# jy0205/Pyramid-Flow

Hardware: NVIDIA H100
Metric: dit_step_latent_tokens_per_sec (higher is better)
Workload: dtype bf16

## Files before the change

pyramid_flow_b200/csrc/pf_attn.cu:

```cuda
#include <algorithm>
#include <vector>

#include "../../include/pf_b200.h"
#include "pf_common.cuh"

namespace pf {

constexpr int ATT_BM = 128;
constexpr int ATT_BN = 128;
constexpr int ATT_HD = 64;
constexpr int ATT_STAGES = 2;
constexpr int ATT_THREADS = 384;
constexpr int ATT_TILE_BYTES = ATT_BN * ATT_HD * 2;
constexpr int ATT_SMEM_BYTES = (1 + 2 * ATT_STAGES) * ATT_TILE_BYTES + 1024;

struct AttnArgs {
  __nv_bfloat16* out;
  long long ldo;
  int batch, heads, seq, q_tiles;
  float scale_log2;
  const int* seg;
  const int* time;
  const int* sched;
  int sched_stride;
  __nv_bfloat16* peer_out[PF_MAX_PEERS];
  int peer_count, peer_chunk_rows, peer_col_begin;
};

__global__ void __launch_bounds__(ATT_THREADS, 1)
attn_fwd_kernel(const __grid_constant__ CUtensorMap tm_q, const __grid_constant__ CUtensorMap tm_k,
                const __grid_constant__ CUtensorMap tm_v, const AttnArgs a) {
  extern __shared__ uint8_t smem_raw[];
  uint8_t* smem = reinterpret_cast<uint8_t*>((reinterpret_cast<uintptr_t>(smem_raw) + 1023) & ~uintptr_t(1023));
  uint8_t* smem_q = smem;
  uint8_t* smem_k = smem + ATT_TILE_BYTES;
  uint8_t* smem_v = smem_k + ATT_STAGES * ATT_TILE_BYTES;

  __shared__ __align__(8) uint64_t bar_q;
  __shared__ __align__(8) uint64_t k_full[ATT_STAGES], k_empty[ATT_STAGES], v_full[ATT_STAGES], v_empty[ATT_STAGES];

  const int warp = threadIdx.x >> 5;
  const int lane = threadIdx.x & 31;
  const int wgroup = warp >> 2;
  const int qt = a.q_tiles - 1 - static_cast<int>(blockIdx.x);
  const int h = blockIdx.y;
  const int b = blockIdx.z;
  const int bh = b * a.heads + h;
  const int* sched = a.sched + (static_cast<size_t>(b) * a.q_tiles + qt) * a.sched_stride;
  const int n_kv = sched[0];

  if (threadIdx.x == 0) {
    tma_prefetch_desc(&tm_q);
    tma_prefetch_desc(&tm_k);
    tma_prefetch_desc(&tm_v);
    mbar_init(&bar_q, 1);
    for (int i = 0; i < ATT_STAGES; ++i) {
      mbar_init(&k_full[i], 1);
      mbar_init(&k_empty[i], 8);
      mbar_init(&v_full[i], 1);
      mbar_init(&v_empty[i], 8);
    }
    fence_barrier_init();
  }
  __syncthreads();

  if (wgroup == 0) {
    setmaxnreg_dec<40>();
    if (warp == 0 && elect_one()) {
      mbar_arrive_expect_tx(&bar_q, ATT_TILE_BYTES);
      tma_load_3d(smem_q, &tm_q, &bar_q, 0, qt * ATT_BM, bh);
      int st = 0;
      uint32_t ph = 0;
      for (int j = 0; j < n_kv; ++j) {
        const int kt = sched[1 + j] >> 1;
        mbar_wait(&k_empty[st], ph ^ 1);
        mbar_arrive_expect_tx(&k_full[st], ATT_TILE_BYTES);
        tma_load_3d(smem_k + st * ATT_TILE_BYTES, &tm_k, &k_full[st], 0, kt * ATT_BN, bh);
        mbar_wait(&v_empty[st], ph ^ 1);
        mbar_arrive_expect_tx(&v_full[st], ATT_TILE_BYTES);
        tma_load_3d(smem_v + st * ATT_TILE_BYTES, &tm_v, &v_full[st], 0, kt * ATT_BN, bh);
        if (++st == ATT_STAGES) {
          st = 0;
          ph ^= 1;
        }
      }
    }
    return;
  }

  setmaxnreg_inc<232>();
  const int wg = wgroup - 1;
  const int g4 = lane >> 2, t4 = lane & 3;
  const int row0 = wg * 64 + (warp & 3) * 16 + g4;
  const float c = a.scale_log2;
  const int* sg = a.seg + static_cast<size_t>(b) * a.seq;
  const int* tm = a.time + static_cast<size_t>(b) * a.seq;
  int seg_q[2], time_q[2];
#pragma unroll
  for (int r = 0; r < 2; ++r) {
    const int qpos = qt * ATT_BM + row0 + 8 * r;
    const bool q_valid = qpos < a.seq;
    seg_q[r] = q_valid ? sg[qpos] : -0x7fffffff;
    time_q[r] = q_valid ? tm[qpos] : -0x7fffffff;
  }
  float m_run[2] = {-INFINITY, -INFINITY};
  float l_run[2] = {0.f, 0.f};
  float o[32];
#pragma unroll
  for (int i = 0; i < 32; ++i) o[i] = 0.f;

  mbar_wait(&bar_q, 0);
  const uint64_t dq = make_smem_desc_kmajor_sw128(smem_u32(smem_q) + wg * (64 * 128));
  int st = 0;
  uint32_t ph = 0;
  for (int j = 0; j < n_kv; ++j) {
    const int entry = sched[1 + j];
    const int kt = entry >> 1;
    const bool masked = (entry & 1) != 0;

    float s[64];
    mbar_wait(&k_full[st], ph);
    {
      const uint64_t dk = make_smem_desc_kmajor_sw128(smem_u32(smem_k + st * ATT_TILE_BYTES));
      wgmma_fence();
#pragma unroll
      for (int kk = 0; kk < ATT_HD / 16; ++kk) wgmma_ss_n128(s, dq + 2 * kk, dk + 2 * kk, kk != 0 ? 1u : 0u);
      wgmma_commit();
      wgmma_wait<0>();
      wgmma_reg_fence(s);
    }
    if (lane == 0) mbar_arrive(&k_empty[st]);

    if (masked) {
#pragma unroll
      for (int i = 0; i < 16; ++i) {
#pragma unroll
        for (int e = 0; e < 2; ++e) {
          const int kv = kt * ATT_BN + 8 * i + 2 * t4 + e;
          int sk = 0x7fffffff, tk = 0x7fffffff;
          if (kv < a.seq) {
            sk = __ldg(sg + kv);
            tk = __ldg(tm + kv);
          }
          if (!(sk == seg_q[0] && tk <= time_q[0])) s[4 * i + e] = -INFINITY;
          if (!(sk == seg_q[1] && tk <= time_q[1])) s[4 * i + 2 + e] = -INFINITY;
        }
      }
    }

    float alpha[2];
#pragma unroll
    for (int r = 0; r < 2; ++r) {
      float mx = -INFINITY;
#pragma unroll
      for (int i = 0; i < 16; ++i) mx = fmaxf(mx, fmaxf(s[4 * i + 2 * r], s[4 * i + 2 * r + 1]));
      mx = fmaxf(mx, __shfl_xor_sync(0xffffffffu, mx, 1));
      mx = fmaxf(mx, __shfl_xor_sync(0xffffffffu, mx, 2));
      const float m_new = fmaxf(m_run[r], mx);
      alpha[r] = (m_new == -INFINITY) ? 1.f : ex2_approx_f((m_run[r] - m_new) * c);
      m_run[r] = m_new;
      const float m_ref = (m_new == -INFINITY) ? 0.f : m_new * c;
      float sum = 0.f;
#pragma unroll
      for (int i = 0; i < 16; ++i) {
        const float p0 = ex2_approx_f(fmaf(s[4 * i + 2 * r], c, -m_ref));
        const float p1 = ex2_approx_f(fmaf(s[4 * i + 2 * r + 1], c, -m_ref));
        s[4 * i + 2 * r] = p0;
        s[4 * i + 2 * r + 1] = p1;
        sum += p0 + p1;
      }
      l_run[r] = l_run[r] * alpha[r] + sum;
    }
#pragma unroll
    for (int i = 0; i < 8; ++i) {
      o[4 * i + 0] *= alpha[0];
      o[4 * i + 1] *= alpha[0];
      o[4 * i + 2] *= alpha[1];
      o[4 * i + 3] *= alpha[1];
    }

    mbar_wait(&v_full[st], ph);
    {
      const uint32_t sv = smem_u32(smem_v + st * ATT_TILE_BYTES);
      uint32_t pa[ATT_BN / 16][4];
#pragma unroll
      for (int kk = 0; kk < ATT_BN / 16; ++kk) {
        pa[kk][0] = pack_bf16x2(s[8 * kk + 0], s[8 * kk + 1]);
        pa[kk][1] = pack_bf16x2(s[8 * kk + 2], s[8 * kk + 3]);
        pa[kk][2] = pack_bf16x2(s[8 * kk + 4], s[8 * kk + 5]);
        pa[kk][3] = pack_bf16x2(s[8 * kk + 6], s[8 * kk + 7]);
      }
      wgmma_reg_fence(o);
      wgmma_fence();
#pragma unroll
      for (int kk = 0; kk < ATT_BN / 16; ++kk) {
        const uint64_t dv = make_smem_desc(sv + kk * 2048, ATT_BN * 128, 1024);
        wgmma_rs_n64_tb(o, pa[kk], dv);
      }
      wgmma_commit();
      wgmma_wait<0>();
      wgmma_reg_fence(o);
    }
    if (lane == 0) mbar_arrive(&v_empty[st]);
    if (++st == ATT_STAGES) {
      st = 0;
      ph ^= 1;
    }
  }

#pragma unroll
  for (int r = 0; r < 2; ++r) {
    float l = l_run[r];
    l += __shfl_xor_sync(0xffffffffu, l, 1);
    l += __shfl_xor_sync(0xffffffffu, l, 2);
    const float inv = (l > 0.f) ? 1.f / l : 0.f;
    const int qpos = qt * ATT_BM + row0 + 8 * r;
    if (qpos >= a.seq) continue;
    __nv_bfloat16* dst;
    if (a.peer_count > 1) {
      const int pr = qpos / a.peer_chunk_rows;
      dst = a.peer_out[pr] + static_cast<size_t>(qpos - pr * a.peer_chunk_rows) * a.ldo + a.peer_col_begin + h * ATT_HD;
    } else {
      dst = a.out + (static_cast<size_t>(b) * a.seq + qpos) * a.ldo + h * ATT_HD;
    }
#pragma unroll
    for (int i = 0; i < 8; ++i)
      *reinterpret_cast<uint32_t*>(dst + 8 * i + 2 * t4) = pack_bf16x2(o[4 * i + 2 * r] * inv, o[4 * i + 2 * r + 1] * inv);
  }
}

int warmup_attn() {
  return ensure_dyn_smem(reinterpret_cast<const void*>(attn_fwd_kernel), ATT_SMEM_BYTES, "attn_fwd_kernel");
}

}

extern "C" int pf_attn_build_schedule(const int32_t* seg, const int32_t* time, int32_t batch, int32_t seq,
                                      int32_t* out, int64_t* allowed_pairs) {
  using namespace pf;
  PF_REQUIRE(batch > 0 && seq > 0, "pf_attn_build_schedule: bad shape");
  const int tiles = (seq + 127) / 128;
  const int stride = 1 + tiles;
  if (out == nullptr) return stride;
  PF_REQUIRE(seg && time, "pf_attn_build_schedule: null ids");
  for (int b = 0; b < batch; ++b) {
    const int32_t* sg = seg + static_cast<size_t>(b) * seq;
    const int32_t* tm = time + static_cast<size_t>(b) * seq;
    std::vector<int32_t> tmin(tiles), tmax(tiles), smin(tiles), smax(tiles);
    for (int t = 0; t < tiles; ++t) {
      const int lo = t * 128, hi = std::min(seq, lo + 128);
      int32_t a = tm[lo], bq = tm[lo], c = sg[lo], d = sg[lo];
      for (int i = lo; i < hi; ++i) {
        a = std::min(a, tm[i]);
        bq = std::max(bq, tm[i]);
        c = std::min(c, sg[i]);
        d = std::max(d, sg[i]);
      }
      tmin[t] = a; tmax[t] = bq; smin[t] = c; smax[t] = d;
    }
    int64_t pairs = 0;
    for (int qt = 0; qt < tiles; ++qt) {
      int32_t* row = out + (static_cast<size_t>(b) * tiles + qt) * stride;
      int cnt = 0;
      const int qlo = qt * 128, qhi = std::min(seq, qlo + 128);
      for (int kt = 0; kt < tiles; ++kt) {
        const int klo = kt * 128, khi = std::min(seq, klo + 128);
        if (tmax[qt] < tmin[kt]) continue;
        if (smax[qt] < smin[kt] || smax[kt] < smin[qt]) continue;
        const bool uniform = (smin[qt] == smax[qt]) && (smin[kt] == smax[kt]) && (smin[qt] == smin[kt]);
        const bool full = uniform && (tmin[qt] >= tmax[kt]) && (khi - klo == 128);
        int64_t n_allowed = 0;
        if (full) {
          n_allowed = static_cast<int64_t>(qhi - qlo) * (khi - klo);
        } else {
          for (int i = qlo; i < qhi; ++i)
            for (int j = klo; j < khi; ++j) n_allowed += (sg[i] == sg[j] && tm[i] >= tm[j]) ? 1 : 0;
          if (n_allowed == 0) continue;
        }
        pairs += n_allowed;
        row[1 + cnt] = (kt << 1) | (full ? 0 : 1);
        ++cnt;
      }
      row[0] = cnt;
      for (int i = 1 + cnt; i < stride; ++i) row[i] = 0;
    }
    if (allowed_pairs) allowed_pairs[b] = pairs;
  }
  return stride;
}

extern "C" int pf_attn_fwd_masked(const pf_attn_desc* d, void* stream_) {
  using namespace pf;
  cudaStream_t stream = static_cast<cudaStream_t>(stream_);
  PF_REQUIRE(d && d->q && d->k && d->v && (d->out || d->peer_count > 1) && d->seg && d->time && d->tile_sched, "pf_attn_fwd_masked: null pointer");
  PF_REQUIRE(d->head_dim == ATT_HD, "pf_attn_fwd_masked: head_dim %d unsupported (64 only)", d->head_dim);
  PF_REQUIRE(d->batch > 0 && d->heads > 0 && d->seq > 0, "pf_attn_fwd_masked: bad shape");
  const int q_tiles = (d->seq + ATT_BM - 1) / ATT_BM;
  PF_REQUIRE(d->sched_stride >= 1 + q_tiles, "pf_attn_fwd_masked: schedule stride %d too small", d->sched_stride);
  PF_REQUIRE(d->q_row_begin >= 0 && d->q_row_begin % ATT_BM == 0 && d->q_row_begin < d->seq,
             "pf_attn_fwd_masked: q_row_begin %d must be a multiple of %d inside the sequence", d->q_row_begin, ATT_BM);
  PF_REQUIRE(d->ldo % 8 == 0 && (reinterpret_cast<uintptr_t>(d->out) & 15) == 0, "pf_attn_fwd_masked: out must be 16-byte aligned");
  PF_REQUIRE(d->variant == 0x10 || d->variant == 0x20 || (d->variant >= 0 && d->variant <= 3), "pf_attn_fwd_masked: bad variant 0x%x", d->variant);
  if (d->variant == 0x20)
    PF_REQUIRE(d->group_sched != nullptr && d->group_mask_index != nullptr && d->group_mask_bits != nullptr,
               "pf_attn_fwd_masked: variant 0x%x needs group_sched, group_mask_index and group_mask_bits", d->variant);
  if (d->variant == 0x10)
    PF_REQUIRE(d->pair_sched != nullptr && d->pair_mask_index != nullptr && d->pair_mask_bits != nullptr,
               "pf_attn_fwd_masked: variant 0x%x needs pair_sched, pair_mask_index and pair_mask_bits", d->variant);
  if (d->peer_count > 1) {
    PF_REQUIRE(d->batch == 1 && d->peer_count <= PF_MAX_PEERS && d->peer_chunk_rows > 0 &&
                   static_cast<long long>(d->peer_chunk_rows) * d->peer_count >= d->seq && d->peer_col_begin % 8 == 0,
               "pf_attn_fwd_masked: bad peer layout (batch %d, count %d, chunk rows %d, seq %d)", d->batch, d->peer_count,
               d->peer_chunk_rows, d->seq);
    for (int i = 0; i < d->peer_count; ++i) PF_REQUIRE(d->peer_out[i] != nullptr, "pf_attn_fwd_masked: peer_out[%d] is null", i);
  }
  CUtensorMap tm[3];
  const void* ptrs[3] = {d->q, d->k, d->v};
  for (int i = 0; i < 3; ++i) {
    const uint64_t dims[3] = {ATT_HD, static_cast<uint64_t>(d->seq), static_cast<uint64_t>(d->batch) * d->heads};
    const uint64_t strides[2] = {ATT_HD * 2, static_cast<uint64_t>(d->seq) * ATT_HD * 2};
    const uint32_t box[3] = {ATT_HD, ATT_BN, 1};
    int rc = encode_tensor_map(&tm[i], CU_TENSOR_MAP_DATA_TYPE_BFLOAT16, 3, ptrs[i], dims, strides, box,
                               CU_TENSOR_MAP_SWIZZLE_128B);
    if (rc) return rc;
  }
  AttnArgs a{};
  a.out = static_cast<__nv_bfloat16*>(d->out);
  a.ldo = d->ldo;
  a.batch = d->batch;
  a.heads = d->heads;
  a.seq = d->seq;
  a.q_tiles = q_tiles;
  a.scale_log2 = d->scale * 1.4426950408889634f;
  a.seg = d->seg;
  a.time = d->time;
  a.sched = d->tile_sched;
  a.sched_stride = d->sched_stride;
  a.peer_count = d->peer_count;
  a.peer_chunk_rows = d->peer_chunk_rows;
  a.peer_col_begin = d->peer_col_begin;
  for (int i = 0; i < PF_MAX_PEERS; ++i) a.peer_out[i] = static_cast<__nv_bfloat16*>(d->peer_out[i]);

  if (int rc = warmup_attn()) return rc;
  dim3 grid(q_tiles - d->q_row_begin / ATT_BM, d->heads, d->batch);
  attn_fwd_kernel<<<grid, ATT_THREADS, ATT_SMEM_BYTES, stream>>>(tm[0], tm[1], tm[2], a);
  return check_launch("pf_attn_fwd_masked");
}
```

pyramid_flow_b200/csrc/pf_common.cuh:

```cuda
#pragma once

#include <cuda.h>
#include <cuda_bf16.h>
#include <cuda_runtime.h>
#include <stdint.h>

namespace pf {

void set_error(const char* fmt, ...);
int  check_launch(const char* what);

#define PF_REQUIRE(cond, ...)                  \
  do {                                         \
    if (!(cond)) {                             \
      ::pf::set_error(__VA_ARGS__);            \
      return -1;                               \
    }                                          \
  } while (0)

int encode_tensor_map(CUtensorMap* map, CUtensorMapDataType dtype, uint32_t rank, const void* base,
                      const uint64_t* dims, const uint64_t* strides_bytes , const uint32_t* box,
                      CUtensorMapSwizzle swizzle,
                      const uint32_t* elem_strides = nullptr );

int num_sms();
int get_option(int key);
int ensure_dyn_smem(const void* kernel, int bytes, const char* what);

__device__ __forceinline__ uint32_t smem_u32(const void* p) {
  return static_cast<uint32_t>(__cvta_generic_to_shared(p));
}

__device__ __forceinline__ bool elect_one() {
  uint32_t pred = 0;
  asm volatile(
      "{\n\t"
      ".reg .b32 %%rx;\n\t"
      ".reg .pred %%px;\n\t"
      "elect.sync %%rx|%%px, 0xffffffff;\n\t"
      "selp.b32 %0, 1, 0, %%px;\n\t"
      "}\n"
      : "=r"(pred));
  return pred != 0;
}

__device__ __forceinline__ void mbar_init(uint64_t* bar, uint32_t count) {
  asm volatile("mbarrier.init.shared::cta.b64 [%0], %1;" ::"r"(smem_u32(bar)), "r"(count) : "memory");
}
__device__ __forceinline__ void fence_barrier_init() {
  asm volatile("fence.mbarrier_init.release.cluster;" ::: "memory");
}
__device__ __forceinline__ void mbar_arrive_expect_tx(uint64_t* bar, uint32_t bytes) {
  asm volatile("mbarrier.arrive.expect_tx.shared::cta.b64 _, [%0], %1;" ::"r"(smem_u32(bar)), "r"(bytes)
               : "memory");
}
__device__ __forceinline__ void mbar_arrive(uint64_t* bar) {
  asm volatile("mbarrier.arrive.shared::cta.b64 _, [%0];" ::"r"(smem_u32(bar)) : "memory");
}
__device__ __forceinline__ bool mbar_try_wait(uint64_t* bar, uint32_t parity) {
  uint32_t ok;
  asm volatile(
      "{\n\t"
      ".reg .pred p;\n\t"
      "mbarrier.try_wait.parity.shared::cta.b64 p, [%1], %2, %3;\n\t"
      "selp.b32 %0, 1, 0, p;\n\t"
      "}\n"
      : "=r"(ok)
      : "r"(smem_u32(bar)), "r"(parity), "r"(0x989680u)
      : "memory");
  return ok != 0;
}
__device__ __forceinline__ bool mbar_test(uint64_t* bar, uint32_t parity) {
  uint32_t ok;
  asm volatile(
      "{\n\t"
      ".reg .pred p;\n\t"
      "mbarrier.test_wait.parity.shared::cta.b64 p, [%1], %2;\n\t"
      "selp.b32 %0, 1, 0, p;\n\t"
      "}\n"
      : "=r"(ok)
      : "r"(smem_u32(bar)), "r"(parity)
      : "memory");
  return ok != 0;
}
__device__ __forceinline__ void mbar_wait(uint64_t* bar, uint32_t parity) {
  while (!mbar_try_wait(bar, parity)) {
  }
}

__device__ __forceinline__ void tma_prefetch_desc(const CUtensorMap* m) {
  asm volatile("prefetch.tensormap [%0];" ::"l"(reinterpret_cast<uint64_t>(m)) : "memory");
}
__device__ __forceinline__ void tma_load_2d(void* smem_dst, const CUtensorMap* m, uint64_t* bar, int c0, int c1) {
  asm volatile(
      "cp.async.bulk.tensor.2d.shared::cluster.global.mbarrier::complete_tx::bytes [%0], [%1, {%3, %4}], [%2];"
      ::"r"(smem_u32(smem_dst)), "l"(reinterpret_cast<uint64_t>(m)), "r"(smem_u32(bar)), "r"(c0), "r"(c1)
      : "memory");
}
__device__ __forceinline__ void tma_load_3d(void* smem_dst, const CUtensorMap* m, uint64_t* bar, int c0, int c1,
                                            int c2) {
  asm volatile(
      "cp.async.bulk.tensor.3d.shared::cluster.global.mbarrier::complete_tx::bytes [%0], [%1, {%3, %4, %5}], [%2];"
      ::"r"(smem_u32(smem_dst)), "l"(reinterpret_cast<uint64_t>(m)), "r"(smem_u32(bar)), "r"(c0), "r"(c1), "r"(c2)
      : "memory");
}
__device__ __forceinline__ void tma_load_4d(void* smem_dst, const CUtensorMap* m, uint64_t* bar, int c0, int c1,
                                            int c2, int c3) {
  asm volatile(
      "cp.async.bulk.tensor.4d.shared::cluster.global.mbarrier::complete_tx::bytes [%0], [%1, {%3, %4, %5, %6}], "
      "[%2];" ::"r"(smem_u32(smem_dst)),
      "l"(reinterpret_cast<uint64_t>(m)), "r"(smem_u32(bar)), "r"(c0), "r"(c1), "r"(c2), "r"(c3)
      : "memory");
}
__device__ __forceinline__ void tma_load_5d(void* smem_dst, const CUtensorMap* m, uint64_t* bar, int c0, int c1,
                                            int c2, int c3, int c4) {
  asm volatile(
      "cp.async.bulk.tensor.5d.shared::cluster.global.mbarrier::complete_tx::bytes [%0], [%1, {%3, %4, %5, %6, "
      "%7}], [%2];" ::"r"(smem_u32(smem_dst)),
      "l"(reinterpret_cast<uint64_t>(m)), "r"(smem_u32(bar)), "r"(c0), "r"(c1), "r"(c2), "r"(c3), "r"(c4)
      : "memory");
}
__device__ __forceinline__ void fence_proxy_async_smem() {
  asm volatile("fence.proxy.async.shared::cta;" ::: "memory");
}
__device__ __forceinline__ void tma_load_2d_multicast(void* smem_dst, const CUtensorMap* m, uint64_t* bar, int c0, int c1,
                                                      uint16_t cta_mask) {
  asm volatile(
      "cp.async.bulk.tensor.2d.shared::cluster.global.mbarrier::complete_tx::bytes.multicast::cluster [%0], [%1, {%3, %4}], "
      "[%2], %5;" ::"r"(smem_u32(smem_dst)),
      "l"(reinterpret_cast<uint64_t>(m)), "r"(smem_u32(bar)), "r"(c0), "r"(c1), "h"(cta_mask)
      : "memory");
}

__device__ __forceinline__ uint32_t cluster_ctarank() {
  uint32_t r;
  asm volatile("mov.u32 %0, %%cluster_ctarank;" : "=r"(r));
  return r;
}
__device__ __forceinline__ void mbar_arrive_cluster(uint64_t* bar, uint32_t cta) {
  asm volatile(
      "{\n\t"
      ".reg .b32 ra;\n\t"
      "mapa.shared::cluster.u32 ra, %0, %1;\n\t"
      "mbarrier.arrive.shared::cluster.b64 _, [ra];\n\t"
      "}\n" ::"r"(smem_u32(bar)), "r"(cta)
      : "memory");
}
__device__ __forceinline__ void cluster_arrive() { asm volatile("barrier.cluster.arrive.release.aligned;" ::: "memory"); }
__device__ __forceinline__ void cluster_wait() { asm volatile("barrier.cluster.wait.acquire.aligned;" ::: "memory"); }

__device__ __forceinline__ void wgmma_fence() { asm volatile("wgmma.fence.sync.aligned;" ::: "memory"); }
__device__ __forceinline__ void wgmma_commit() { asm volatile("wgmma.commit_group.sync.aligned;" ::: "memory"); }
template <int N>
__device__ __forceinline__ void wgmma_wait() {
  asm volatile("wgmma.wait_group.sync.aligned %0;" ::"n"(N) : "memory");
}
template <int N>
__device__ __forceinline__ void wgmma_reg_fence(float (&d)[N]) {
#pragma unroll
  for (int i = 0; i < N; ++i) asm volatile("" : "+f"(d[i])::"memory");
}
template <int REGS>
__device__ __forceinline__ void setmaxnreg_inc() {
  asm volatile("setmaxnreg.inc.sync.aligned.u32 %0;" ::"n"(REGS));
}
template <int REGS>
__device__ __forceinline__ void setmaxnreg_dec() {
  asm volatile("setmaxnreg.dec.sync.aligned.u32 %0;" ::"n"(REGS));
}
__device__ __forceinline__ void named_bar_sync(int id, int threads) {
  asm volatile("bar.sync %0, %1;" ::"r"(id), "r"(threads) : "memory");
}

__device__ __forceinline__ void wgmma_ss_n128(float (&d)[64], uint64_t desc_a, uint64_t desc_b, uint32_t accumulate) {
  asm volatile(
      "{\n\t"
      ".reg .pred p;\n\t"
      "setp.ne.b32 p, %66, 0;\n\t"
      "wgmma.mma_async.sync.aligned.m64n128k16.f32.bf16.bf16 "
      "{%0, %1, %2, %3, %4, %5, %6, %7, %8, %9, %10, %11, %12, %13, %14, %15, %16, %17, %18, %19, %20, %21, %22, %23, %24, %25, %26, %27, %28, %29, %30, %31, %32, %33, %34, %35, %36, %37, %38, %39, %40, %41, %42, %43, %44, %45, %46, %47, %48, %49, %50, %51, %52, %53, %54, %55, %56, %57, %58, %59, %60, %61, %62, %63}, %64, %65, p, 1, 1, 0, 0;\n\t"
      "}\n"
      : "+f"(d[0]), "+f"(d[1]), "+f"(d[2]), "+f"(d[3]), "+f"(d[4]), "+f"(d[5]), "+f"(d[6]), "+f"(d[7]), "+f"(d[8]), "+f"(d[9]), "+f"(d[10]), "+f"(d[11]), "+f"(d[12]), "+f"(d[13]), "+f"(d[14]), "+f"(d[15]), "+f"(d[16]), "+f"(d[17]), "+f"(d[18]), "+f"(d[19]), "+f"(d[20]), "+f"(d[21]), "+f"(d[22]), "+f"(d[23]), "+f"(d[24]), "+f"(d[25]), "+f"(d[26]), "+f"(d[27]), "+f"(d[28]), "+f"(d[29]), "+f"(d[30]), "+f"(d[31]), "+f"(d[32]), "+f"(d[33]), "+f"(d[34]), "+f"(d[35]), "+f"(d[36]), "+f"(d[37]), "+f"(d[38]), "+f"(d[39]), "+f"(d[40]), "+f"(d[41]), "+f"(d[42]), "+f"(d[43]), "+f"(d[44]), "+f"(d[45]), "+f"(d[46]), "+f"(d[47]), "+f"(d[48]), "+f"(d[49]), "+f"(d[50]), "+f"(d[51]), "+f"(d[52]), "+f"(d[53]), "+f"(d[54]), "+f"(d[55]), "+f"(d[56]), "+f"(d[57]), "+f"(d[58]), "+f"(d[59]), "+f"(d[60]), "+f"(d[61]), "+f"(d[62]), "+f"(d[63])
      : "l"(desc_a), "l"(desc_b), "r"(accumulate)
      : "memory");
}
__device__ __forceinline__ void wgmma_ss_n128_e4m3(float (&d)[64], uint64_t desc_a, uint64_t desc_b, uint32_t accumulate) {
  asm volatile(
      "{\n\t"
      ".reg .pred p;\n\t"
      "setp.ne.b32 p, %66, 0;\n\t"
      "wgmma.mma_async.sync.aligned.m64n128k32.f32.e4m3.e4m3 "
      "{%0, %1, %2, %3, %4, %5, %6, %7, %8, %9, %10, %11, %12, %13, %14, %15, %16, %17, %18, %19, %20, %21, %22, %23, %24, %25, %26, %27, %28, %29, %30, %31, %32, %33, %34, %35, %36, %37, %38, %39, %40, %41, %42, %43, %44, %45, %46, %47, %48, %49, %50, %51, %52, %53, %54, %55, %56, %57, %58, %59, %60, %61, %62, %63}, %64, %65, p, 1, 1;\n\t"
      "}\n"
      : "+f"(d[0]), "+f"(d[1]), "+f"(d[2]), "+f"(d[3]), "+f"(d[4]), "+f"(d[5]), "+f"(d[6]), "+f"(d[7]), "+f"(d[8]), "+f"(d[9]), "+f"(d[10]), "+f"(d[11]), "+f"(d[12]), "+f"(d[13]), "+f"(d[14]), "+f"(d[15]), "+f"(d[16]), "+f"(d[17]), "+f"(d[18]), "+f"(d[19]), "+f"(d[20]), "+f"(d[21]), "+f"(d[22]), "+f"(d[23]), "+f"(d[24]), "+f"(d[25]), "+f"(d[26]), "+f"(d[27]), "+f"(d[28]), "+f"(d[29]), "+f"(d[30]), "+f"(d[31]), "+f"(d[32]), "+f"(d[33]), "+f"(d[34]), "+f"(d[35]), "+f"(d[36]), "+f"(d[37]), "+f"(d[38]), "+f"(d[39]), "+f"(d[40]), "+f"(d[41]), "+f"(d[42]), "+f"(d[43]), "+f"(d[44]), "+f"(d[45]), "+f"(d[46]), "+f"(d[47]), "+f"(d[48]), "+f"(d[49]), "+f"(d[50]), "+f"(d[51]), "+f"(d[52]), "+f"(d[53]), "+f"(d[54]), "+f"(d[55]), "+f"(d[56]), "+f"(d[57]), "+f"(d[58]), "+f"(d[59]), "+f"(d[60]), "+f"(d[61]), "+f"(d[62]), "+f"(d[63])
      : "l"(desc_a), "l"(desc_b), "r"(accumulate)
      : "memory");
}
__device__ __forceinline__ void wgmma_ss_n64(float (&d)[32], uint64_t desc_a, uint64_t desc_b, uint32_t accumulate) {
  asm volatile(
      "{\n\t"
      ".reg .pred p;\n\t"
      "setp.ne.b32 p, %34, 0;\n\t"
      "wgmma.mma_async.sync.aligned.m64n64k16.f32.bf16.bf16 "
      "{%0, %1, %2, %3, %4, %5, %6, %7, %8, %9, %10, %11, %12, %13, %14, %15, %16, %17, %18, %19, %20, %21, %22, %23, %24, %25, %26, %27, %28, %29, %30, %31}, %32, %33, p, 1, 1, 0, 0;\n\t"
      "}\n"
      : "+f"(d[0]), "+f"(d[1]), "+f"(d[2]), "+f"(d[3]), "+f"(d[4]), "+f"(d[5]), "+f"(d[6]), "+f"(d[7]), "+f"(d[8]), "+f"(d[9]), "+f"(d[10]), "+f"(d[11]), "+f"(d[12]), "+f"(d[13]), "+f"(d[14]), "+f"(d[15]), "+f"(d[16]), "+f"(d[17]), "+f"(d[18]), "+f"(d[19]), "+f"(d[20]), "+f"(d[21]), "+f"(d[22]), "+f"(d[23]), "+f"(d[24]), "+f"(d[25]), "+f"(d[26]), "+f"(d[27]), "+f"(d[28]), "+f"(d[29]), "+f"(d[30]), "+f"(d[31])
      : "l"(desc_a), "l"(desc_b), "r"(accumulate)
      : "memory");
}
__device__ __forceinline__ void wgmma_rs_n64_tb(float (&d)[32], const uint32_t (&a)[4], uint64_t desc_b) {
  asm volatile(
      "{\n\t"
      ".reg .pred p;\n\t"
      "setp.ne.b32 p, 1, 0;\n\t"
      "wgmma.mma_async.sync.aligned.m64n64k16.f32.bf16.bf16 "
      "{%0, %1, %2, %3, %4, %5, %6, %7, %8, %9, %10, %11, %12, %13, %14, %15, %16, %17, %18, %19, %20, %21, %22, %23, %24, %25, %26, %27, %28, %29, %30, %31}, {%32, %33, %34, %35}, %36, p, 1, 1, 1;\n\t"
      "}\n"
      : "+f"(d[0]), "+f"(d[1]), "+f"(d[2]), "+f"(d[3]), "+f"(d[4]), "+f"(d[5]), "+f"(d[6]), "+f"(d[7]), "+f"(d[8]), "+f"(d[9]), "+f"(d[10]), "+f"(d[11]), "+f"(d[12]), "+f"(d[13]), "+f"(d[14]), "+f"(d[15]), "+f"(d[16]), "+f"(d[17]), "+f"(d[18]), "+f"(d[19]), "+f"(d[20]), "+f"(d[21]), "+f"(d[22]), "+f"(d[23]), "+f"(d[24]), "+f"(d[25]), "+f"(d[26]), "+f"(d[27]), "+f"(d[28]), "+f"(d[29]), "+f"(d[30]), "+f"(d[31])
      : "r"(a[0]), "r"(a[1]), "r"(a[2]), "r"(a[3]), "l"(desc_b)
      : "memory");
}
template <int BN>
__device__ __forceinline__ void wgmma_ss(float (&d)[BN / 2], uint64_t desc_a, uint64_t desc_b, uint32_t accumulate) {
  static_assert(BN == 128 || BN == 64, "wgmma_ss: tile widths 128 and 64 are instantiated");
  if constexpr (BN == 128) wgmma_ss_n128(d, desc_a, desc_b, accumulate);
  else wgmma_ss_n64(d, desc_a, desc_b, accumulate);
}

__device__ __forceinline__ uint64_t make_smem_desc(uint32_t saddr, uint32_t lbo_bytes, uint32_t sbo_bytes) {
  uint64_t d = 0;
  d |= static_cast<uint64_t>((saddr & 0x3FFFFu) >> 4);
  d |= static_cast<uint64_t>((lbo_bytes >> 4) & 0x3FFFu) << 16;
  d |= static_cast<uint64_t>((sbo_bytes >> 4) & 0x3FFFu) << 32;
  d |= static_cast<uint64_t>(1) << 62;
  return d;
}
__device__ __forceinline__ uint64_t make_smem_desc_kmajor_sw128(uint32_t saddr) {
  return make_smem_desc(saddr, 16, 1024);
}

constexpr int PIPE_THREADS = 384;
constexpr int PIPE_CONSUMER_WARPS = 8;
constexpr int PIPE_BM = 128;
constexpr int PIPE_BK = 64;
template <int BN>
struct PipeCfg {
  static constexpr int A_BYTES = PIPE_BM * PIPE_BK * 2;
  static constexpr int B_BYTES = BN * PIPE_BK * 2;
  static constexpr int STAGE_BYTES = A_BYTES + B_BYTES;
  static constexpr int STAGES = (BN >= 128) ? 4 : 6;
  static constexpr int ACC_PITCH = BN + 8;
  static constexpr int ACC_BYTES = PIPE_BM * ACC_PITCH * 4;
  static constexpr int SMEM_BYTES = STAGES * STAGE_BYTES + ACC_BYTES + 1024;
};

template <int BN>
__device__ __forceinline__ void pipe_consume_tile(float (&acc)[BN / 2], uint8_t* smem, uint64_t* full_bar, uint64_t* empty_bar,
                                                  int num_kb, int wg, int& stage, uint32_t& phase) {
  using Cfg = PipeCfg<BN>;
  const int lane = threadIdx.x & 31;
  int prev = -1;
  for (int kb = 0; kb < num_kb; ++kb) {
    mbar_wait(&full_bar[stage], phase);
    const uint32_t sa = smem_u32(smem + stage * Cfg::STAGE_BYTES);
    const uint64_t da = make_smem_desc_kmajor_sw128(sa + wg * (64 * 128));
    const uint64_t db = make_smem_desc_kmajor_sw128(sa + Cfg::A_BYTES);
    wgmma_reg_fence(acc);
    wgmma_fence();
#pragma unroll
    for (int kk = 0; kk < PIPE_BK / 16; ++kk) wgmma_ss<BN>(acc, da + 2 * kk, db + 2 * kk, (kb | kk) != 0 ? 1u : 0u);
    wgmma_commit();
    wgmma_wait<1>();
    if (prev >= 0 && lane == 0) mbar_arrive(&empty_bar[prev]);
    prev = stage;
    if (++stage == Cfg::STAGES) {
      stage = 0;
      phase ^= 1;
    }
  }
  wgmma_wait<0>();
  wgmma_reg_fence(acc);
  if (prev >= 0 && lane == 0) mbar_arrive(&empty_bar[prev]);
}

template <int BN>
__device__ __forceinline__ void pipe_stage_acc(const float (&acc)[BN / 2], float* acc_tile, int wg) {
  const int w = (threadIdx.x >> 5) & 3, lane = threadIdx.x & 31;
  float* r0 = acc_tile + (wg * 64 + w * 16 + (lane >> 2)) * PipeCfg<BN>::ACC_PITCH + 2 * (lane & 3);
  float* r1 = r0 + 8 * PipeCfg<BN>::ACC_PITCH;
#pragma unroll
  for (int i = 0; i < BN / 8; ++i) {
    *reinterpret_cast<float2*>(r0 + 8 * i) = make_float2(acc[4 * i + 0], acc[4 * i + 1]);
    *reinterpret_cast<float2*>(r1 + 8 * i) = make_float2(acc[4 * i + 2], acc[4 * i + 3]);
  }
}

__device__ __forceinline__ uint32_t pack_bf16x2(float lo, float hi) {
  __nv_bfloat162 v = __floats2bfloat162_rn(lo, hi);
  return *reinterpret_cast<uint32_t*>(&v);
}
__device__ __forceinline__ float rcp_approx_f(float x) {
  float y;
  asm("rcp.approx.ftz.f32 %0, %1;" : "=f"(y) : "f"(x));
  return y;
}
__device__ __forceinline__ float ex2_approx_f(float x) {
  float y;
  asm("ex2.approx.ftz.f32 %0, %1;" : "=f"(y) : "f"(x));
  return y;
}
__device__ __forceinline__ float gelu_tanh_f(float x) {
  const float c0 = -2.0f * 0.7978845608028654f * 1.4426950408889634f;
  const float c1 = c0 * 0.044715f;
  const float x2 = x * x;
  const float nu = x * fmaf(x2, c1, c0);
  return x * rcp_approx_f(1.0f + ex2_approx_f(nu));
}
__device__ __forceinline__ float silu_f(float x) {
  return x * rcp_approx_f(1.0f + ex2_approx_f(-1.4426950408889634f * x));
}

}
```

Before: 126,900.

## Software-pipeline attention QK and PV wgmma with ping-pong warpgroup scheduling

Restructures the attention KV loop so the QK^T wgmma for tile j is issued together with the PV wgmma for tile j-1, overlapping tensor-core work with the softmax of the previous tile, FA3-style. Named barriers make the two consumer warpgroups take turns issuing MMAs, so one warpgroup's softmax runs while the other's GEMMs execute. KV pipeline stages go from 2 to 3 so K(j+1) and V(j) can be resident at once. This costs more shared memory and register pressure (s, pa and o are live together), and adds more complex barrier and phase bookkeeping.

```diff
diff --git a/pyramid_flow_b200/csrc/pf_attn.cu b/pyramid_flow_b200/csrc/pf_attn.cu
--- a/pyramid_flow_b200/csrc/pf_attn.cu
+++ b/pyramid_flow_b200/csrc/pf_attn.cu
@@ -9,10 +9,18 @@
 constexpr int ATT_BM = 128;
 constexpr int ATT_BN = 128;
 constexpr int ATT_HD = 64;
-constexpr int ATT_STAGES = 2;
+constexpr int ATT_STAGES = 3;
 constexpr int ATT_THREADS = 384;
 constexpr int ATT_TILE_BYTES = ATT_BN * ATT_HD * 2;
 constexpr int ATT_SMEM_BYTES = (1 + 2 * ATT_STAGES) * ATT_TILE_BYTES + 1024;
+static_assert(ATT_STAGES >= 2, "the kv loop keeps K(j) and V(j - 1) in flight at once");
+
+__device__ __forceinline__ void reg_fence_u32(uint32_t (&a)[ATT_BN / 16][4]) {
+#pragma unroll
+  for (int i = 0; i < ATT_BN / 16; ++i)
+#pragma unroll
+    for (int k = 0; k < 4; ++k) asm volatile("" : "+r"(a[i][k])::"memory");
+}
 
 struct AttnArgs {
   __nv_bfloat16* out;
@@ -111,27 +119,29 @@
 
   mbar_wait(&bar_q, 0);
   const uint64_t dq = make_smem_desc_kmajor_sw128(smem_u32(smem_q) + wg * (64 * 128));
-  int st = 0;
-  uint32_t ph = 0;
-  for (int j = 0; j < n_kv; ++j) {
-    const int entry = sched[1 + j];
-    const int kt = entry >> 1;
-    const bool masked = (entry & 1) != 0;
-
-    float s[64];
-    mbar_wait(&k_full[st], ph);
-    {
-      const uint64_t dk = make_smem_desc_kmajor_sw128(smem_u32(smem_k + st * ATT_TILE_BYTES));
-      wgmma_fence();
-#pragma unroll
-      for (int kk = 0; kk < ATT_HD / 16; ++kk) wgmma_ss_n128(s, dq + 2 * kk, dk + 2 * kk, kk != 0 ? 1u : 0u);
-      wgmma_commit();
-      wgmma_wait<0>();
-      wgmma_reg_fence(s);
-    }
-    if (lane == 0) mbar_arrive(&k_empty[st]);
-
-    if (masked) {
+
+  auto issue_qk = [&](float (&s)[64], int stage) {
+    const uint64_t dk = make_smem_desc_kmajor_sw128(smem_u32(smem_k + stage * ATT_TILE_BYTES));
+    wgmma_reg_fence(s);
+    wgmma_fence();
+#pragma unroll
+    for (int kk = 0; kk < ATT_HD / 16; ++kk) wgmma_ss_n128(s, dq + 2 * kk, dk + 2 * kk, kk != 0 ? 1u : 0u);
+    wgmma_commit();
+  };
+  auto issue_pv = [&](const uint32_t (&pa)[ATT_BN / 16][4], int stage) {
+    const uint32_t sv = smem_u32(smem_v + stage * ATT_TILE_BYTES);
+    wgmma_reg_fence(o);
+    wgmma_fence();
+#pragma unroll
+    for (int kk = 0; kk < ATT_BN / 16; ++kk) {
+      const uint64_t dv = make_smem_desc(sv + kk * 2048, ATT_BN * 128, 1024);
+      wgmma_rs_n64_tb(o, pa[kk], dv);
+    }
+    wgmma_commit();
+  };
+  auto softmax = [&](float (&s)[64], int entry, float (&alpha)[2]) {
+    if ((entry & 1) != 0) {
+      const int kt = entry >> 1;
 #pragma unroll
       for (int i = 0; i < 16; ++i) {
 #pragma unroll
@@ -147,8 +157,6 @@
         }
       }
     }
-
-    float alpha[2];
 #pragma unroll
     for (int r = 0; r < 2; ++r) {
       float mx = -INFINITY;
@@ -171,6 +179,8 @@
       }
       l_run[r] = l_run[r] * alpha[r] + sum;
     }
+  };
+  auto rescale_pack = [&](const float (&s)[64], const float (&alpha)[2], uint32_t (&pa)[ATT_BN / 16][4]) {
 #pragma unroll
     for (int i = 0; i < 8; ++i) {
       o[4 * i + 0] *= alpha[0];
@@ -178,34 +188,71 @@
       o[4 * i + 2] *= alpha[1];
       o[4 * i + 3] *= alpha[1];
     }
-
-    mbar_wait(&v_full[st], ph);
-    {
-      const uint32_t sv = smem_u32(smem_v + st * ATT_TILE_BYTES);
-      uint32_t pa[ATT_BN / 16][4];
-#pragma unroll
-      for (int kk = 0; kk < ATT_BN / 16; ++kk) {
-        pa[kk][0] = pack_bf16x2(s[8 * kk + 0], s[8 * kk + 1]);
-        pa[kk][1] = pack_bf16x2(s[8 * kk + 2], s[8 * kk + 3]);
-        pa[kk][2] = pack_bf16x2(s[8 * kk + 4], s[8 * kk + 5]);
-        pa[kk][3] = pack_bf16x2(s[8 * kk + 6], s[8 * kk + 7]);
-      }
-      wgmma_reg_fence(o);
-      wgmma_fence();
-#pragma unroll
-      for (int kk = 0; kk < ATT_BN / 16; ++kk) {
-        const uint64_t dv = make_smem_desc(sv + kk * 2048, ATT_BN * 128, 1024);
-        wgmma_rs_n64_tb(o, pa[kk], dv);
-      }
-      wgmma_commit();
+#pragma unroll
+    for (int kk = 0; kk < ATT_BN / 16; ++kk) {
+      pa[kk][0] = pack_bf16x2(s[8 * kk + 0], s[8 * kk + 1]);
+      pa[kk][1] = pack_bf16x2(s[8 * kk + 2], s[8 * kk + 3]);
+      pa[kk][2] = pack_bf16x2(s[8 * kk + 4], s[8 * kk + 5]);
+      pa[kk][3] = pack_bf16x2(s[8 * kk + 6], s[8 * kk + 7]);
+    }
+  };
+
+  if (n_kv > 0) {
+    float s[64];
+    uint32_t pa[ATT_BN / 16][4];
+    float alpha[2];
+
+    const int bar_mine = 1 + wg, bar_other = 2 - wg;
+    if (wg == 1) named_bar_arrive(1, 256);
+
+    mbar_wait(&k_full[0], 0);
+    named_bar_sync(bar_mine, 256);
+    issue_qk(s, 0);
+    named_bar_arrive(bar_other, 256);
+    wgmma_wait<0>();
+    wgmma_reg_fence(s);
+    if (lane == 0) mbar_arrive(&k_empty[0]);
+    softmax(s, sched[1], alpha);
+
+    int st = 0;
+    uint32_t ph = 0;
+    int st_retire = -1;
+    for (int j = 1; j < n_kv; ++j) {
       wgmma_wait<0>();
       wgmma_reg_fence(o);
-    }
+      reg_fence_u32(pa);
+      if (st_retire >= 0 && lane == 0) mbar_arrive(&v_empty[st_retire]);
+      rescale_pack(s, alpha, pa);
+      const int st_k = (st + 1 == ATT_STAGES) ? 0 : st + 1;
+      const uint32_t ph_k = (st + 1 == ATT_STAGES) ? ph ^ 1 : ph;
+      mbar_wait(&k_full[st_k], ph_k);
+      mbar_wait(&v_full[st], ph);
+      named_bar_sync(bar_mine, 256);
+      issue_qk(s, st_k);
+      issue_pv(pa, st);
+      named_bar_arrive(bar_other, 256);
+      wgmma_wait<1>();
+      wgmma_reg_fence(s);
+      if (lane == 0) mbar_arrive(&k_empty[st_k]);
+      softmax(s, sched[1 + j], alpha);
+      st_retire = st;
+      st = st_k;
+      ph = ph_k;
+    }
+
+    wgmma_wait<0>();
+    wgmma_reg_fence(o);
+    reg_fence_u32(pa);
+    if (st_retire >= 0 && lane == 0) mbar_arrive(&v_empty[st_retire]);
+    rescale_pack(s, alpha, pa);
+    mbar_wait(&v_full[st], ph);
+    named_bar_sync(bar_mine, 256);
+    issue_pv(pa, st);
+    if (wg == 0) named_bar_arrive(bar_other, 256);
+    wgmma_wait<0>();
+    wgmma_reg_fence(o);
+    reg_fence_u32(pa);
     if (lane == 0) mbar_arrive(&v_empty[st]);
-    if (++st == ATT_STAGES) {
-      st = 0;
-      ph ^= 1;
-    }
   }
 
 #pragma unroll
diff --git a/pyramid_flow_b200/csrc/pf_common.cuh b/pyramid_flow_b200/csrc/pf_common.cuh
--- a/pyramid_flow_b200/csrc/pf_common.cuh
+++ b/pyramid_flow_b200/csrc/pf_common.cuh
@@ -170,6 +170,9 @@
 }
 __device__ __forceinline__ void named_bar_sync(int id, int threads) {
   asm volatile("bar.sync %0, %1;" ::"r"(id), "r"(threads) : "memory");
+}
+__device__ __forceinline__ void named_bar_arrive(int id, int threads) {
+  asm volatile("bar.arrive %0, %1;" ::"r"(id), "r"(threads) : "memory");
 }
 
 __device__ __forceinline__ void wgmma_ss_n128(float (&d)[64], uint64_t desc_a, uint64_t desc_b, uint32_t accumulate) {
```

New measurement: 129,100 (median of 6 runs). +1.7%, better.

## Software-pipeline attention QK/PV and ping-pong schedule the two consumer warpgroups

Applied to the files above, without the earlier changes.

Restructures the attention main loop so that the PV GEMM for the previous KV tile and the QK GEMM for the next tile are issued in one wgmma burst, with softmax running between bursts. Two consumer warpgroups alternate via named barriers (bar.sync/bar.arrive) so that one warpgroup's tensor-core burst overlaps the other's softmax. The aim is to hide exp/mask work behind tensor-core execution. In exchange, separate K and V stage/phase counters are kept, S and the packed P live across iterations (adding register pressure), and the barrier handoff has a subtle tail case.

```diff
diff --git a/pyramid_flow_b200/csrc/pf_attn.cu b/pyramid_flow_b200/csrc/pf_attn.cu
--- a/pyramid_flow_b200/csrc/pf_attn.cu
+++ b/pyramid_flow_b200/csrc/pf_attn.cu
@@ -1,4 +1,5 @@
 #include <algorithm>
+#include <type_traits>
 #include <vector>
 
 #include "../../include/pf_b200.h"
@@ -111,25 +112,58 @@
 
   mbar_wait(&bar_q, 0);
   const uint64_t dq = make_smem_desc_kmajor_sw128(smem_u32(smem_q) + wg * (64 * 128));
-  int st = 0;
-  uint32_t ph = 0;
-  for (int j = 0; j < n_kv; ++j) {
+
+  const int own_bar = 1 + wg, other_bar = 2 - wg;
+  float s[64];
+  uint32_t pa[ATT_BN / 16][4];
+  int kst = 0, vst = 0;
+  uint32_t kph = 0, vph = 0;
+
+  auto burst = [&](auto pv, auto qk, bool pass_turn) {
+    constexpr bool PV = decltype(pv)::value, QK = decltype(qk)::value;
+    if constexpr (PV) mbar_wait(&v_full[vst], vph);
+    if constexpr (QK) mbar_wait(&k_full[kst], kph);
+    named_bar_sync(own_bar, 256);
+    if constexpr (PV) wgmma_reg_fence(o);
+    wgmma_fence();
+    if constexpr (PV) {
+      const uint32_t sv = smem_u32(smem_v + vst * ATT_TILE_BYTES);
+#pragma unroll
+      for (int kk = 0; kk < ATT_BN / 16; ++kk) {
+        const uint64_t dv = make_smem_desc(sv + kk * 2048, ATT_BN * 128, 1024);
+        wgmma_rs_n64_tb(o, pa[kk], dv);
+      }
+    }
+    if constexpr (QK) {
+      const uint64_t dk = make_smem_desc_kmajor_sw128(smem_u32(smem_k + kst * ATT_TILE_BYTES));
+#pragma unroll
+      for (int kk = 0; kk < ATT_HD / 16; ++kk) wgmma_ss_n128(s, dq + 2 * kk, dk + 2 * kk, kk != 0 ? 1u : 0u);
+    }
+    wgmma_commit();
+    if (pass_turn) named_bar_arrive(other_bar, 256);
+    wgmma_wait<0>();
+    if constexpr (PV) {
+      wgmma_reg_fence(o);
+      if (lane == 0) mbar_arrive(&v_empty[vst]);
+      if (++vst == ATT_STAGES) {
+        vst = 0;
+        vph ^= 1;
+      }
+    }
+    if constexpr (QK) {
+      wgmma_reg_fence(s);
+      if (lane == 0) mbar_arrive(&k_empty[kst]);
+      if (++kst == ATT_STAGES) {
+        kst = 0;
+        kph ^= 1;
+      }
+    }
+  };
+
+  auto softmax = [&](int j) {
     const int entry = sched[1 + j];
     const int kt = entry >> 1;
     const bool masked = (entry & 1) != 0;
-
-    float s[64];
-    mbar_wait(&k_full[st], ph);
-    {
-      const uint64_t dk = make_smem_desc_kmajor_sw128(smem_u32(smem_k + st * ATT_TILE_BYTES));
-      wgmma_fence();
-#pragma unroll
-      for (int kk = 0; kk < ATT_HD / 16; ++kk) wgmma_ss_n128(s, dq + 2 * kk, dk + 2 * kk, kk != 0 ? 1u : 0u);
-      wgmma_commit();
-      wgmma_wait<0>();
-      wgmma_reg_fence(s);
-    }
-    if (lane == 0) mbar_arrive(&k_empty[st]);
 
     if (masked) {
 #pragma unroll
@@ -178,34 +212,24 @@
       o[4 * i + 2] *= alpha[1];
       o[4 * i + 3] *= alpha[1];
     }
-
-    mbar_wait(&v_full[st], ph);
-    {
-      const uint32_t sv = smem_u32(smem_v + st * ATT_TILE_BYTES);
-      uint32_t pa[ATT_BN / 16][4];
-#pragma unroll
-      for (int kk = 0; kk < ATT_BN / 16; ++kk) {
-        pa[kk][0] = pack_bf16x2(s[8 * kk + 0], s[8 * kk + 1]);
-        pa[kk][1] = pack_bf16x2(s[8 * kk + 2], s[8 * kk + 3]);
-        pa[kk][2] = pack_bf16x2(s[8 * kk + 4], s[8 * kk + 5]);
-        pa[kk][3] = pack_bf16x2(s[8 * kk + 6], s[8 * kk + 7]);
-      }
-      wgmma_reg_fence(o);
-      wgmma_fence();
-#pragma unroll
-      for (int kk = 0; kk < ATT_BN / 16; ++kk) {
-        const uint64_t dv = make_smem_desc(sv + kk * 2048, ATT_BN * 128, 1024);
-        wgmma_rs_n64_tb(o, pa[kk], dv);
-      }
-      wgmma_commit();
-      wgmma_wait<0>();
-      wgmma_reg_fence(o);
-    }
-    if (lane == 0) mbar_arrive(&v_empty[st]);
-    if (++st == ATT_STAGES) {
-      st = 0;
-      ph ^= 1;
-    }
+#pragma unroll
+    for (int kk = 0; kk < ATT_BN / 16; ++kk) {
+      pa[kk][0] = pack_bf16x2(s[8 * kk + 0], s[8 * kk + 1]);
+      pa[kk][1] = pack_bf16x2(s[8 * kk + 2], s[8 * kk + 3]);
+      pa[kk][2] = pack_bf16x2(s[8 * kk + 4], s[8 * kk + 5]);
+      pa[kk][3] = pack_bf16x2(s[8 * kk + 6], s[8 * kk + 7]);
+    }
+  };
+
+  if (n_kv > 0) {
+    if (wg == 1) named_bar_arrive(1, 256);
+    burst(std::false_type{}, std::true_type{}, true);
+    for (int j = 1; j < n_kv; ++j) {
+      softmax(j - 1);
+      burst(std::true_type{}, std::true_type{}, true);
+    }
+    softmax(n_kv - 1);
+    burst(std::true_type{}, std::false_type{}, wg == 0);
   }
 
 #pragma unroll
diff --git a/pyramid_flow_b200/csrc/pf_common.cuh b/pyramid_flow_b200/csrc/pf_common.cuh
--- a/pyramid_flow_b200/csrc/pf_common.cuh
+++ b/pyramid_flow_b200/csrc/pf_common.cuh
@@ -170,6 +170,9 @@
 }
 __device__ __forceinline__ void named_bar_sync(int id, int threads) {
   asm volatile("bar.sync %0, %1;" ::"r"(id), "r"(threads) : "memory");
+}
+__device__ __forceinline__ void named_bar_arrive(int id, int threads) {
+  asm volatile("bar.arrive %0, %1;" ::"r"(id), "r"(threads) : "memory");
 }
 
 __device__ __forceinline__ void wgmma_ss_n128(float (&d)[64], uint64_t desc_a, uint64_t desc_b, uint32_t accumulate) {
```

Measured after the change: 123,900 before, 127,100 after (median of 6 runs). 1.03x the previous value.
